# Ryan-Yanlong/DREAM-GNN

Hardware: AMD Instinct MI355X
Metric: GCMC+FGCN SpMM edges/sec and achieved HBM GB/s at 1/2/4/8 MI355X (higher is better)
Workload: dtype f32

## Files before the change

### dream_gnn_amd/csrc/dgmi_api.hip

```cpp
#include <hip/hip_runtime.h>
#include <limits.h>
#include <stdlib.h>
#include <string.h>

#include "dgmi.h"
#include "dgmi_bf16.h"
#include "dgmi_keep.h"
#include "dgmi_kernels.h"
#include "dgmi_tuning.h"

namespace {

inline hipStream_t as_stream(dgmi_stream_t s) { return static_cast<hipStream_t>(s); }

inline int from_hip(hipError_t e) { return e == hipSuccess ? DGMI_OK : DGMI_ERR_LAUNCH; }

long long env_ll(const char* name, long long dflt) {
  const char* e = getenv(name);
  return e != nullptr && e[0] != '\0' ? atoll(e) : dflt;
}

}

namespace dgmi {

Tuning& tuning() {
  static Tuning t = [] {
    Tuning v;
    v.sliced_rows = (int)env_ll("DGMI_SLICED_ROWS", 0);
    v.sliced_touch_lead = (int)env_ll("DGMI_SLICED_PF", -1);
    v.sliced_lpr = (int)env_ll("DGMI_SLICED_LPR", 0);
    v.sliced_no_off32 = getenv("DGMI_NO_OFF32") != nullptr ? 1 : 0;
    v.sliced_chunk_rows = env_ll("DGMI_SLICED_CHUNK_ROWS", 0);
    v.sliced_taper_rows = env_ll("DGMI_SLICED_TAPER_ROWS", 0);
    v.sliced_owned = (int)env_ll("DGMI_SLICED_OWNED", -1);
    v.sliced_owned_grid = (int)env_ll("DGMI_SLICED_OWNED_GRID", 0);
    v.sliced_owned_wgs = (int)env_ll("DGMI_SLICED_OWNED_WGS", 0);
    v.sliced_owned_rows = (int)env_ll("DGMI_SLICED_OWNED_ROWS", 0);
    v.sliced_owned_lds_rows = env_ll("DGMI_SLICED_OWNED_LDS_ROWS", 0);
    v.sliced_owned_lag = (int)env_ll("DGMI_SLICED_OWNED_LAG", -2);
    v.sliced_owned_spin_ticks = env_ll("DGMI_SLICED_OWNED_SPIN_TICKS", 0);
    v.select_window_min = env_ll("DGMI_SELECT_WINDOW_MIN", 0);
    v.select_narrow_window = env_ll("DGMI_SELECT_NARROW_WINDOW", 0) != 0 ? 1 : 0;
    v.sort_plain_tiles = env_ll("DGMI_SORT_PLAIN_TILES", 0) != 0 ? 1 : 0;
    v.knn_screen_first = env_ll("DGMI_KNN_SCREEN_V1", 0) != 0 ? 1 : 0;
    v.knn_pool_chunks = env_ll("DGMI_KNN_POOL_CHUNKS", 0);
    return v;
  }();
  return t;
}

}

extern "C" {

DGMI_API int dgmi_set_tuning(const char* name, int64_t value) {
  if (name == nullptr) return DGMI_ERR_INVALID_ARG;
  dgmi::Tuning& t = dgmi::tuning();
  if (strcmp(name, "sliced_rows") == 0) t.sliced_rows = (int)value;
  else if (strcmp(name, "sliced_touch_lead") == 0) t.sliced_touch_lead = (int)value;
  else if (strcmp(name, "sliced_lpr") == 0) t.sliced_lpr = (int)value;
  else if (strcmp(name, "sliced_no_off32") == 0) t.sliced_no_off32 = value != 0;
  else if (strcmp(name, "sliced_chunk_rows") == 0) t.sliced_chunk_rows = value;
  else if (strcmp(name, "sliced_taper_rows") == 0) t.sliced_taper_rows = value;
  else if (strcmp(name, "sliced_owned") == 0) t.sliced_owned = (int)value;
  else if (strcmp(name, "sliced_owned_grid") == 0) t.sliced_owned_grid = (int)value;
  else if (strcmp(name, "sliced_owned_wgs") == 0) t.sliced_owned_wgs = (int)value;
  else if (strcmp(name, "sliced_owned_rows") == 0) t.sliced_owned_rows = (int)value;
  else if (strcmp(name, "sliced_owned_lds_rows") == 0) t.sliced_owned_lds_rows = value;
  else if (strcmp(name, "sliced_owned_lag") == 0) t.sliced_owned_lag = (int)value;
  else if (strcmp(name, "sliced_owned_spin_ticks") == 0) t.sliced_owned_spin_ticks = value;
  else if (strcmp(name, "select_window_min") == 0) t.select_window_min = value;
  else if (strcmp(name, "select_narrow_window") == 0) t.select_narrow_window = value != 0;
  else if (strcmp(name, "sort_plain_tiles") == 0) t.sort_plain_tiles = value != 0;
  else if (strcmp(name, "knn_screen_first") == 0) t.knn_screen_first = value != 0;
  else if (strcmp(name, "knn_pool_chunks") == 0) t.knn_pool_chunks = value;
  else return DGMI_ERR_INVALID_ARG;
  return DGMI_OK;
}

DGMI_API int dgmi_abi_version(void) { return DGMI_ABI_VERSION; }

DGMI_API const char* dgmi_status_string(int status) {
  switch (status) {
    case DGMI_OK: return "ok";
    case DGMI_ERR_INVALID_ARG: return "invalid argument (null pointer, negative size or ld < F)";
    case DGMI_ERR_TOO_LARGE: return "size does not fit the int32 id space";
    case DGMI_ERR_WORKSPACE: return "workspace missing or too small";
    case DGMI_ERR_LAUNCH: return "HIP launch failed";
    case DGMI_ERR_NO_DEVICE: return "no gfx950 device visible";
    default: return "unknown dgmi status";
  }
}

DGMI_API int dgmi_device_ok(void) {
  int n = 0;
  if (hipGetDeviceCount(&n) != hipSuccess || n <= 0) return 0;
  int dev = 0;
  if (hipGetDevice(&dev) != hipSuccess) return 0;
  hipDeviceProp_t prop;
  if (hipGetDeviceProperties(&prop, dev) != hipSuccess) return 0;
  return strncmp(prop.gcnArchName, "gfx950", 6) == 0 ? 1 : 0;
}

DGMI_API int dgmi_csr_from_coo_i32(const int32_t* row, const int32_t* col, int64_t E, int64_t n_rows,
                          int64_t n_cols, int32_t* indptr, int32_t* indices, int32_t* eid, void* workspace,
                          size_t* workspace_bytes, dgmi_stream_t stream) {
  if (E < 0 || n_rows < 0 || workspace_bytes == nullptr) return DGMI_ERR_INVALID_ARG;
  if (E > INT32_MAX || n_rows >= INT32_MAX || n_cols >= INT32_MAX) return DGMI_ERR_TOO_LARGE;
  if (workspace != nullptr) {
    if (indptr == nullptr) return DGMI_ERR_INVALID_ARG;
    if (E > 0 && (row == nullptr || col == nullptr || indices == nullptr || eid == nullptr))
      return DGMI_ERR_INVALID_ARG;
  }
  size_t need = 0;
  hipError_t err = dgmi::csr_from_coo_i32(row, col, E, n_rows, n_cols, indptr, indices, eid, nullptr,
                                          &need, as_stream(stream));
  if (err != hipSuccess) return DGMI_ERR_LAUNCH;
  if (workspace == nullptr) {
    *workspace_bytes = need;
    return DGMI_OK;
  }
  if (*workspace_bytes < need) return DGMI_ERR_WORKSPACE;
  return from_hip(dgmi::csr_from_coo_i32(row, col, E, n_rows, n_cols, indptr, indices, eid, workspace,
                                         workspace_bytes, as_stream(stream)));
}

static bool epilogue_ok(int32_t act, const float* out_mask, int64_t ld_mask, int64_t F) {
  return (act == 0 || act == 1) && (out_mask == nullptr || ld_mask >= F);
}

static bool keep_args_ok(const int32_t* eid, const uint32_t* keep, int32_t n_keep) {
  if (n_keep < 0 || n_keep > dgmi::kMaxKeepSegs) return false;
  return n_keep == 0 || (eid != nullptr && keep != nullptr);
}

DGMI_API int dgmi_spmm_csr_f32(const int32_t* indptr, const int32_t* indices, const float* vals,
                      const int32_t* eid, const uint32_t* keep, int32_t n_keep,
                      const float* X, int64_t ldx, const float* src_scale,
                      const float* dst_scale, float* Y, int64_t ldy, int64_t n_dst,
                      int64_t n_src, int64_t F, int32_t act, float act_slope, const float* out_mask,
                      int64_t ld_mask, float out_mask_scale, dgmi_stream_t stream) {
  if (n_dst < 0 || n_src < 0 || F < 0 || !keep_args_ok(eid, keep, n_keep) || !epilogue_ok(act, out_mask, ld_mask, F))
    return DGMI_ERR_INVALID_ARG;
  if (n_dst >= INT32_MAX || n_src >= INT32_MAX || F > INT32_MAX) return DGMI_ERR_TOO_LARGE;
  if (n_dst == 0 || F == 0) return DGMI_OK;
  if (indptr == nullptr || Y == nullptr) return DGMI_ERR_INVALID_ARG;
  if (ldx < F || ldy < F) return DGMI_ERR_INVALID_ARG;
  if (X == nullptr && n_src > 0) return DGMI_ERR_INVALID_ARG;
  if (static_cast<const void*>(X) == static_cast<const void*>(Y)) return DGMI_ERR_INVALID_ARG;
  dgmi::SpmmArgs a{indptr, indices, vals, X, ldx, src_scale, dst_scale, Y, ldy, n_dst, n_src, F,
                   nullptr, 0, 0, nullptr, 0, eid, keep, n_keep, {act, act_slope, out_mask, ld_mask, out_mask_scale}};
  return from_hip(dgmi::spmm_csr_f32(a, as_stream(stream)));
}

DGMI_API int32_t dgmi_spmm_default_chunk(int64_t n_rows, int64_t nnz) {
  (void)n_rows;
  int64_t c = (nnz / 4096 + 63) / 64 * 64;
  if (c < 64) c = 64;
  if (c > 512) c = 512;
  return (int32_t)c;
}

static bool chunk_ok(int32_t chunk) { return chunk >= 16 && chunk <= 65536; }

DGMI_API size_t dgmi_spmm_plan_bytes(int64_t n_rows, int64_t nnz, int32_t chunk) {
  if (n_rows < 0 || nnz < 0 || !chunk_ok(chunk)) return 0;
  return dgmi::plan_bytes(n_rows, nnz, chunk);
}

DGMI_API size_t dgmi_spmm_partials_bytes(int64_t nnz, int32_t chunk, int64_t F) {
  if (nnz < 0 || F < 0 || !chunk_ok(chunk)) return 0;
  const size_t ldp = (size_t)((F + 3) / 4 * 4);
  const size_t b = (size_t)dgmi::plan_slots_cap(nnz, chunk) * ldp * sizeof(float);
  return b < 16 ? 16 : b;
}

DGMI_API int dgmi_spmm_plan_build(const int32_t* indptr, int64_t n_rows, int64_t nnz, int32_t chunk,
                                  void* plan, size_t plan_bytes, void* workspace,
                                  size_t* workspace_bytes, dgmi_stream_t stream) {
  if (n_rows < 0 || nnz < 0 || !chunk_ok(chunk) || workspace_bytes == nullptr)
    return DGMI_ERR_INVALID_ARG;
  if (n_rows >= INT32_MAX || nnz > INT32_MAX) return DGMI_ERR_TOO_LARGE;
  size_t need = 0;
  if (dgmi::spmm_plan_build(indptr, n_rows, nnz, chunk, nullptr, nullptr, &need, as_stream(stream)) !=
      hipSuccess)
    return DGMI_ERR_LAUNCH;
  if (workspace == nullptr) {
    *workspace_bytes = need;
    return DGMI_OK;
  }
  if (plan == nullptr || (indptr == nullptr && n_rows > 0)) return DGMI_ERR_INVALID_ARG;
  if (*workspace_bytes < need || plan_bytes < dgmi::plan_bytes(n_rows, nnz, chunk))
    return DGMI_ERR_WORKSPACE;
  return from_hip(dgmi::spmm_plan_build(indptr, n_rows, nnz, chunk, static_cast<int32_t*>(plan),
                                        workspace, workspace_bytes, as_stream(stream)));
}

DGMI_API int dgmi_spmm_csr_planned_f32(const int32_t* indptr, const int32_t* indices,
                                       const float* vals, const int32_t* eid, const uint32_t* keep,
                                       int32_t n_keep, const float* X, int64_t ldx,
                                       const float* src_scale, const float* dst_scale, float* Y,
                                       int64_t ldy, int64_t n_dst, int64_t n_src, int64_t F,
                                       int64_t nnz, int32_t chunk, const void* plan, void* partials,
                                       size_t partials_bytes, int32_t act, float act_slope,
                                       const float* out_mask, int64_t ld_mask, float out_mask_scale,
                                       dgmi_stream_t stream) {
  if (n_dst < 0 || n_src < 0 || F < 0 || nnz < 0 || !chunk_ok(chunk) || !keep_args_ok(eid, keep, n_keep) ||
      !epilogue_ok(act, out_mask, ld_mask, F))
    return DGMI_ERR_INVALID_ARG;
  if (n_dst >= INT32_MAX || n_src >= INT32_MAX || F > INT32_MAX || nnz > INT32_MAX)
    return DGMI_ERR_TOO_LARGE;
  if (n_dst == 0 || F == 0) return DGMI_OK;
  if (indptr == nullptr || Y == nullptr || plan == nullptr || partials == nullptr)
    return DGMI_ERR_INVALID_ARG;
  if (ldx < F || ldy < F) return DGMI_ERR_INVALID_ARG;
  if (X == nullptr && n_src > 0) return DGMI_ERR_INVALID_ARG;
  if (static_cast<const void*>(X) == static_cast<const void*>(Y)) return DGMI_ERR_INVALID_ARG;
  if (partials_bytes < dgmi_spmm_partials_bytes(nnz, chunk, F)) return DGMI_ERR_WORKSPACE;
  dgmi::SpmmArgs a{indptr, indices, vals, X, ldx, src_scale, dst_scale, Y, ldy, n_dst, n_src, F,
                   static_cast<const int32_t*>(plan), nnz, chunk, static_cast<float*>(partials),
                   (F + 3) / 4 * 4, eid, keep, n_keep, {act, act_slope, out_mask, ld_mask, out_mask_scale}};
// ... 336 lines not shown
```

### dream_gnn_amd/csrc/dgmi_owned.hip

```cpp
#include <hip/hip_runtime.h>
#include <stdint.h>

#include <map>
#include <mutex>
#include <utility>

#include "dgmi_owned_common.h"
#include "dgmi_sliced_common.h"

namespace dgmi {
namespace {

constexpr int kOwnedTouchChunk = 4;
constexpr int kOwnedTouchLead = 8;
constexpr int64_t kOwnedSpinTicks = 3000;
constexpr int64_t kOwnedMinRows = 32768;
constexpr int kOwnedLag = -1;

struct OwnedWork {
  int phase, task, slice, col_round;
  int64_t row0;
  int lds_row, rows;
};

__device__ __forceinline__ OwnedWork owned_decode(const OwnedPlan& pl, int64_t wg, int T, int k, int grp) {
  OwnedWork w;
  w.phase = k / T;
  w.task = k - w.phase * T;
  const OwnedPhase ph = owned_phase(pl, w.phase);
  w.slice = ph.slice;
  w.col_round = ph.col_round;
  const OwnedTask t = owned_task(pl, wg, ph.row_round, w.task, grp);
  w.row0 = t.row0;
  w.lds_row = t.lds_row;
  w.rows = t.rows;
  return w;
}

template <int LPR, int VALS, bool OFF32, int WAVES>
__global__ __launch_bounds__(kWave* WAVES, WAVES == kOwnedWaves ? 4 : 6) void spmm_owned_kernel(
    const int32_t* __restrict__ segptr, const int32_t* __restrict__ indices, const float* __restrict__ X, int64_t ldx,
    const float* __restrict__ dst_scale, float* __restrict__ Y, int64_t ldy, int64_t n_dst, int F, OwnedPlan pl,
    unsigned* __restrict__ arrive, int lag, int64_t spin_ticks, Epilogue ep) {
  constexpr bool MULT = VALS == 2;
  constexpr int kIdMask = MULT ? (int)kMultIdMask : 0x7fffffff;
  extern __shared__ float4 lds_rows[];
  const int lane = threadIdx.x & (kWave - 1);
  const int wave = threadIdx.x >> 6;
  const int grp = lane / LPR, glane = lane % LPR, gbase = grp * LPR;
  const int64_t wg = blockIdx.x;
  const int T = owned_wg_tasks(pl, wg);
  if (T == 0) return;
  int* done = reinterpret_cast<int*>(lds_rows + (size_t)pl.round_rows * LPR);
  int* phase_cnt = done + pl.tasks;
  int* counter = phase_cnt + pl.phases;
  int* open = counter + 1;
  for (int i = threadIdx.x; i < pl.tasks + pl.phases + 2; i += blockDim.x) done[i] = 0;
  __syncthreads();
  const int total = pl.phases * T;
  const int label = (int)(blockIdx.x & 7u);

  if (wave == WAVES - 1) {
    const unsigned n_label = (unsigned)((pl.active - label + 7) >> 3);
    const unsigned* my_arrive = arrive + (size_t)label * pl.phases;
    const int chunks_per_phase = (T + kOwnedTouchChunk - 1) / kOwnedTouchChunk, chunks = pl.phases * chunks_per_phase;
    const int last_gate = lag >= 0 ? pl.phases - 1 : 0;
    int keepalive = 0, touched = 0, opened = 0;
    bool waiting = false;
    uint64_t wait_start = 0;
    while (touched < chunks || opened < last_gate) {
      bool idle = true;
      const int next = __hip_atomic_load(counter, __ATOMIC_RELAXED, __HIP_MEMORY_SCOPE_WORKGROUP);
      if (touched < chunks) {
        const int P = touched / chunks_per_phase, t0 = (touched - P * chunks_per_phase) * kOwnedTouchChunk;
        if (P * T + t0 <= next + kOwnedTouchLead) {
          ++touched;
          idle = false;
          const OwnedPhase ph = owned_phase(pl, P);
          const int64_t in_round = owned_round_rows(pl, wg, ph.row_round);
          const int64_t lds_first = (int64_t)t0 * pl.G * pl.R;
          int64_t lds_last = lds_first + (int64_t)kOwnedTouchChunk * pl.G * pl.R;
          if (lds_last > in_round) lds_last = in_round;
          if (lds_first < lds_last) {
            const int32_t* sp_s = segptr + (int64_t)ph.slice * n_dst;
            const int64_t r_first = owned_task(pl, wg, ph.row_round, t0, 0).row0, r_last = r_first + (lds_last - lds_first);
            const int64_t rp = lane == 0 ? r_first : (lane == 1 ? r_last : r_first + (int64_t)(lane - 1) * 32);
            int v = 0;
            if (rp <= r_last) v = sp_s[rp];
            keepalive ^= v;
            const int e0 = __builtin_amdgcn_readlane(v, 0), e1 = __builtin_amdgcn_readlane(v, 1);
            for (int64_t p = (int64_t)e0 + (int64_t)lane * 32; p < e1; p += (int64_t)kWave * 32) keepalive ^= indices[p];
            asm volatile("" ::"v"(keepalive));
          }
        }
      }
      if (opened < last_gate) {
        const int P = opened + 1, need = P - 1 - lag;
        bool ok = need < 0 || __hip_atomic_load(&my_arrive[need], __ATOMIC_RELAXED, __HIP_MEMORY_SCOPE_AGENT) >= n_label;
        if (!ok && next >= P * T) {
          const uint64_t now = __builtin_amdgcn_s_memrealtime();
          if (!waiting) {
            waiting = true;
            wait_start = now;
          } else if (now - wait_start >= (uint64_t)spin_ticks) {
            ok = true;
          }
        }
        if (ok) {
          opened = P;
          waiting = false;
          idle = false;
          __hip_atomic_store(open, P, __ATOMIC_RELAXED, __HIP_MEMORY_SCOPE_WORKGROUP);
        }
      }
      if (idle) __builtin_amdgcn_s_sleep(2);
    }
    return;
  }

  auto grab = [&]() {
    int k = 0;
    if (lane == 0) k = __hip_atomic_fetch_add(counter, 1, __ATOMIC_RELAXED, __HIP_MEMORY_SCOPE_WORKGROUP);
    return __builtin_amdgcn_readfirstlane(k);
  };
  auto boundaries = [&](int k) {
    if (k >= total) return 0;
    const OwnedWork w = owned_decode(pl, wg, T, k, grp);
    if (w.rows == 0) return 0;
    return segptr[(int64_t)w.slice * n_dst + w.row0 + (glane < w.rows ? glane : w.rows)];
  };
  auto first_ids = [&](int my_b, int rows, int batch) {
    const int e_begin = __shfl(my_b, gbase, kWave), e_end = __shfl(my_b, gbase + rows, kWave);
    if (rows == 0 || e_begin >= e_end) return 0;
    return indices[e_begin + owned_window_id_edge(batch, glane, e_end - e_begin)];
  };
  static_assert(kOwnedWindowFirstBatches == 2, "nxt_idx and nxt_idx1");

  const uint32_t row_bytes = (uint32_t)ldx * 4u;
  int k = grab();
  int my_b = boundaries(k);
  int nxt_idx = k < total ? first_ids(my_b, owned_decode(pl, wg, T, k, grp).rows, 0) : 0;
  int nxt_idx1 = k < total ? first_ids(my_b, owned_decode(pl, wg, T, k, grp).rows, 1) : 0;
  while (k < total) {
    const OwnedWork w = owned_decode(pl, wg, T, k, grp);
    const int k_next = grab();
    const int next_b = boundaries(k_next);
    if (lag >= 0)
      while (__hip_atomic_load(open, __ATOMIC_RELAXED, __HIP_MEMORY_SCOPE_WORKGROUP) < w.phase) __builtin_amdgcn_s_sleep(1);
    while (__hip_atomic_load(&done[w.task], __ATOMIC_ACQUIRE, __HIP_MEMORY_SCOPE_WORKGROUP) < w.phase) __builtin_amdgcn_s_sleep(1);

    const int nr = w.rows;
    int col = (w.col_round * LPR + glane) * 4;
    const bool col_ok = col < F;
    if (!col_ok) col = 0;
    const float* Xc = X + col;
    const uint32_t col_bytes = (uint32_t)col * 4u;
    float4* slot = lds_rows + (size_t)w.lds_row * LPR + glane;
    auto commit = [&](int r, const float4& acc) {
      if (w.slice == 0) {
        slot[r * LPR] = acc;
        return;
      }
      float4 t = slot[r * LPR];
      t.x += acc.x;
      t.y += acc.y;
      t.z += acc.z;
      t.w += acc.w;
      slot[r * LPR] = t;
    };
    auto write_rows = [&]() {
      if (w.slice != kOwnedSlices - 1 || !col_ok) return;
      for (int r = 0; r < nr; ++r) {
        float4 t = slot[r * LPR];
        const int64_t row = w.row0 + r;
        if (dst_scale != nullptr) {
          const float d = dst_scale[row];
          t.x *= d;
          t.y *= d;
          t.z *= d;
          t.w *= d;
        }
        *reinterpret_cast<float4*>(Y + row * ldy + col) = epilogue4(ep, t, row, col);
      }
    };

    if (nr > 0) {
      const int e_begin = __shfl(my_b, gbase, kWave);
      const int e_end = __shfl(my_b, gbase + nr, kWave);
      int r = 0;
      int row_end = __shfl(my_b, gbase + 1, kWave);
      float4 acc = make_float4(0.f, 0.f, 0.f, 0.f);
      if (e_begin < e_end) {
        constexpr int W = kOwnedWindow;
        static_assert(W <= 8 && kMultShift == 28 && LPR % W == 0, "at most eight 4-bit multiplicity fields, shifted down from bit 28");
        const int L = e_end - e_begin;
        float4 v[W];
        int idx[W];
        uint32_t mults = 0, mults_in = 0;
        auto read_ids = [&](int batch_idx) {
#pragma unroll
          for (int u = 0; u < W; ++u) {
            int id = __shfl(batch_idx, gbase + u, kWave);
            if (MULT) {
              mults_in = (mults_in >> 4) | ((uint32_t)id & ((uint32_t)kMultMax << kMultShift));
              id &= kIdMask;
            }
            idx[u] = id;
          }
          if (MULT) asm volatile("" : "+v"(mults_in));
        };
        auto add = [&](int u) {
          if (MULT) {
            const float m = (float)(((mults >> (32 - 4 * W)) & (uint32_t)kMultMax) + 1u);
            mults >>= 4;
            acc.x = fmaf(m, v[u].x, acc.x);
            acc.y = fmaf(m, v[u].y, acc.y);
            acc.z = fmaf(m, v[u].z, acc.z);
            acc.w = fmaf(m, v[u].w, acc.w);
          } else {
            acc.x += v[u].x;
            acc.y += v[u].y;
            acc.z += v[u].z;
            acc.w += v[u].w;
          }
        };
        auto rows_before = [&](int p) {
          while (p >= row_end) {
            commit(r, acc);
            acc = make_float4(0.f, 0.f, 0.f, 0.f);
            ++r;
            row_end = __shfl(my_b, gbase + r + 1, kWave);
          }
        };
        read_ids(nxt_idx);
        int ids = nxt_idx1;
#pragma unroll
        for (int u = 0; u < W; ++u) v[u] = ld_row<OFF32>(X, Xc, idx[u], ldx, row_bytes, col_bytes);
        mults = mults_in;
        __builtin_amdgcn_sched_barrier(0);
        int p0 = e_begin;
        for (int g = 0; p0 + W < e_end; ++g, p0 += W) {
          read_ids(ids);
          ids = indices[e_begin + owned_window_id_edge(owned_window_request_batch(g), glane, L)];
          __builtin_amdgcn_sched_barrier(0);
#pragma unroll
          for (int u = 0; u < W; ++u) {
            rows_before(p0 + u);
            add(u);
            v[u] = ld_row<OFF32>(X, Xc, idx[u], ldx, row_bytes, col_bytes);
            __builtin_amdgcn_sched_barrier(0);
          }
          mults = mults_in;
        }
#pragma unroll
        for (int u = 0; u < W; ++u) {
          if (p0 + u < e_end) {
            rows_before(p0 + u);
            add(u);
          }
        }
      }
      for (; r < nr; ++r) {
        commit(r, acc);
        acc = make_float4(0.f, 0.f, 0.f, 0.f);
      }
      write_rows();
    }
    nxt_idx = k_next < total ? first_ids(next_b, owned_decode(pl, wg, T, k_next, grp).rows, 0) : 0;
    nxt_idx1 = k_next < total ? first_ids(next_b, owned_decode(pl, wg, T, k_next, grp).rows, 1) : 0;
    __builtin_amdgcn_wave_barrier();
    if (lane == 0) {
      __hip_atomic_store(&done[w.task], w.phase + 1, __ATOMIC_RELEASE, __HIP_MEMORY_SCOPE_WORKGROUP);
      if (lag >= 0) {
        const int finished = __hip_atomic_fetch_add(&phase_cnt[w.phase], 1, __ATOMIC_RELAXED, __HIP_MEMORY_SCOPE_WORKGROUP);
        if (finished == T - 1)
          __hip_atomic_fetch_add(&arrive[(size_t)label * pl.phases + w.phase], 1u, __ATOMIC_RELAXED, __HIP_MEMORY_SCOPE_AGENT);
      }
    }
    k = k_next;
    my_b = next_b;
  }
}

int device_cus() {
  static const int cus = [] {
    int dev = 0, n = 0;
    if (hipGetDevice(&dev) != hipSuccess || hipDeviceGetAttribute(&n, hipDeviceAttributeMultiprocessorCount, dev) != hipSuccess)
      return 0;
    return n;
  }();
  return cus;
}

int owned_class_form(const OwnedPlan& pl, bool id_mult, int64_t table_bytes) {
  const auto mib = [&](int64_t lo, int64_t hi) { return table_bytes >= (lo << 20) && table_bytes <= (hi << 20); };
  if (pl.col_rounds == 1 && pl.row_rounds == 2 && !id_mult && mib(16, 32)) return 1;
  if (pl.col_rounds == 2 && pl.row_rounds == 1 && id_mult && mib(48, 64)) return 1;
  if (pl.col_rounds == 1 && pl.row_rounds == 1 && id_mult && mib(16, 32)) return 1;
  return 0;
}

bool owned_coresident(const void* kern, int threads, size_t lds, int wgs) {
  static std::mutex mu;
  static std::map<std::pair<const void*, size_t>, int> known;
  std::lock_guard<std::mutex> lock(mu);
  auto it = known.find({kern, lds});
  if (it == known.end()) {
    int n = 0;
    if (hipOccupancyMaxActiveBlocksPerMultiprocessor(&n, kern, threads, lds) != hipSuccess) {
      (void)hipGetLastError();
      n = 0;
    }
    it = known.emplace(std::make_pair(kern, lds), n).first;
  }
  return it->second >= wgs;
}

template <int LPR, int WAVES>
hipError_t launch_owned(const SlicedArgs& a, const OwnedPlan& pl, int64_t grid, bool off32, int lag, int64_t spin_ticks,
                        hipStream_t s, bool* resident) {
  constexpr int kWgsPerCu = WAVES == kOwnedWaves ? 1 : 2;
  unsigned* arrive = reinterpret_cast<unsigned*>(a.planes);
  *resident = true;
#define DGMI_OWNED(V, O)                                                                                                  \
  do {                                                                                                                    \
    if constexpr (kWgsPerCu > 1 && LPR == 8 && V == 2) {                                                                  \
      *resident = false;                                                                                                  \
      return hipSuccess;                                                                                                  \
    } else {                                                                                                              \
    auto kern = spmm_owned_kernel<LPR, V, O, WAVES>;                                                                      \
    static const hipError_t attr = hipFuncSetAttribute(reinterpret_cast<const void*>(kern),                               \
                                                       hipFuncAttributeMaxDynamicSharedMemorySize, (160 << 10) / kWgsPerCu); \
    if (attr != hipSuccess) return attr;                                                                                  \
    if (kWgsPerCu > 1 && !owned_coresident(reinterpret_cast<const void*>(kern), kWave * WAVES, pl.lds_bytes, kWgsPerCu)) { \
      *resident = false;                                                                                                  \
      return hipSuccess;                                                                                                  \
    }                                                                                                                     \
    if (lag >= 0) {                                                            \
      const hipError_t err = hipMemsetAsync(arrive, 0, sizeof(unsigned) * 8 * (size_t)pl.phases, s);                      \
      if (err != hipSuccess) return err;                                                                                  \
    }                                                                                                                     \
    hipLaunchKernelGGL(kern, dim3((unsigned)grid), dim3(kWave* WAVES), pl.lds_bytes, s, a.segptr, a.indices,              \
                       static_cast<const float*>(a.X), a.ldx, a.dst_scale, a.Y, a.ldy, a.n_dst, (int)a.F, pl, arrive, lag, \
                       spin_ticks, a.ep);                                                                                 \
    }                                                                                                                     \
  } while (0)
  if (a.id_mult) {
    if (off32) DGMI_OWNED(2, true); else DGMI_OWNED(2, false);
  } else {
    if (off32) DGMI_OWNED(0, true); else DGMI_OWNED(0, false);
  }
#undef DGMI_OWNED
  return hipGetLastError();
}

}

hipError_t spmm_owned_try(const SlicedArgs& a, hipStream_t s, bool* taken) {
  *taken = false;
  const Tuning& tune = tuning();
  if (tune.sliced_owned == 0) return hipSuccess;
  if (a.x_bytes != 4 || a.vals != nullptr || a.src_scale != nullptr || a.n_keep != 0 || a.n_slices != kOwnedSlices ||
      tune.sliced_chunk_rows > 0 || a.chunk_rows < a.n_dst || a.n_dst == 0 || a.F == 0)
    return hipSuccess;
  const int64_t grid = tune.sliced_owned_grid > 0 ? tune.sliced_owned_grid : device_cus();
  if (grid < 1) return hipSuccess;
  const int lpr = sliced_lpr(a.F, a.n_src, a.n_slices, a.n_dst, a.full_width, a.n_keep, a.x_bytes, tune.sliced_lpr);
  const OwnedPlan pl = owned_plan(a.n_dst, a.F, lpr, grid, tune.sliced_owned_rows, tune.sliced_owned_lds_rows);
  if (!pl.ok || pl.lds_bytes > (size_t)(160 << 10)) return hipSuccess;
  const auto arrive_fits = [&](const OwnedPlan& p) {
    return sizeof(unsigned) * 8 * (size_t)p.phases <= sizeof(float) * (size_t)a.n_slices * (size_t)a.n_dst * (size_t)a.ldp;
  };
  if (!arrive_fits(pl)) return hipSuccess;
  const int rule = a.n_dst < kOwnedMinRows ? 0 : owned_class_form(pl, a.id_mult, a.n_src * a.ldx * (int64_t)sizeof(float));
  if (tune.sliced_owned != 1 && rule == 0) return hipSuccess;
  const int form = tune.sliced_owned_wgs == 1 || tune.sliced_owned_wgs == 2 ? tune.sliced_owned_wgs : (rule == 2 ? 2 : 1);
  const bool off32 = !tune.sliced_no_off32 && (a.n_src * a.ldx + a.F) * 4 < ((int64_t)1 << 32);
  const int64_t spin = tune.sliced_owned_spin_ticks > 0 ? tune.sliced_owned_spin_ticks : kOwnedSpinTicks;
  const int lag = tune.sliced_owned_lag >= -1 ? tune.sliced_owned_lag : kOwnedLag;
  *taken = true;
  bool resident = true;
  if (form == 2) {
    const int64_t grid2 = tune.sliced_owned_grid > 0 ? grid : 2 * grid;
    const OwnedPlan pl2 = owned_plan(a.n_dst, a.F, lpr, grid2, tune.sliced_owned_rows, tune.sliced_owned_lds_rows, 2);
    if (pl2.ok && pl2.lds_bytes <= (size_t)(80 << 10) && arrive_fits(pl2)) {
      hipError_t err;
      switch (lpr) {
        case 8: err = launch_owned<8, kOwnedPairWaves>(a, pl2, grid2, off32, lag, spin, s, &resident); break;
        case 16: err = launch_owned<16, kOwnedPairWaves>(a, pl2, grid2, off32, lag, spin, s, &resident); break;
        case 32: err = launch_owned<32, kOwnedPairWaves>(a, pl2, grid2, off32, lag, spin, s, &resident); break;
        default: err = launch_owned<64, kOwnedPairWaves>(a, pl2, grid2, off32, lag, spin, s, &resident); break;
      }
      if (err != hipSuccess || resident) return err;
    }
  }
  switch (lpr) {
    case 8: return launch_owned<8, kOwnedWaves>(a, pl, grid, off32, lag, spin, s, &resident);
    case 16: return launch_owned<16, kOwnedWaves>(a, pl, grid, off32, lag, spin, s, &resident);
    case 32: return launch_owned<32, kOwnedWaves>(a, pl, grid, off32, lag, spin, s, &resident);
    default: return launch_owned<64, kOwnedWaves>(a, pl, grid, off32, lag, spin, s, &resident);
  }
}

}
```

### dream_gnn_amd/csrc/dgmi_owned_common.h

```cpp
#pragma once
#include <hip/hip_runtime.h>
#include <stddef.h>
#include <stdint.h>

namespace dgmi {

constexpr int kOwnedSlices = 8;
constexpr int kOwnedWaves = 16;
constexpr int kOwnedWorkers = kOwnedWaves - 1;
constexpr int kOwnedPairWaves = 12;
constexpr int64_t kOwnedLdsRowBytes = 144 << 10;
constexpr int kOwnedMaxPhases = 128;
constexpr int kOwnedPhaseTasks = 24;
constexpr int kOwnedMaxRows = 8;

struct OwnedPlan {
  bool ok;
  int lpr, G, R;
  int col_rounds, row_rounds, phases;
  int64_t wg_rows;
  int64_t active;
  int round_rows;
  int tasks;
  int64_t n_dst;
  size_t lds_bytes;
};

struct OwnedPhase {
  int col_round, row_round, slice;
};

struct OwnedTask {
  int64_t row0;
  int lds_row;
  int rows;
};

__host__ __device__ constexpr int owned_form_waves(int wgs_per_cu) { return wgs_per_cu == 2 ? kOwnedPairWaves : kOwnedWaves; }

__host__ __device__ inline OwnedPlan owned_plan(int64_t n_dst, int64_t F, int lpr, int64_t grid, int R_req, int64_t lds_rows_cap,
                                                int wgs_per_cu = 1) {
  OwnedPlan p{};
  p.ok = false;
  p.n_dst = n_dst;
  if (n_dst < 1 || F < 1 || grid < 1 || (wgs_per_cu != 1 && wgs_per_cu != 2) || (lpr != 8 && lpr != 16 && lpr != 32 && lpr != 64)) return p;
  p.lpr = lpr;
  p.G = 64 / lpr;
  p.col_rounds = (int)((F + 4 * lpr - 1) / (4 * lpr));
  p.wg_rows = (n_dst + grid - 1) / grid;
  p.active = (n_dst + p.wg_rows - 1) / p.wg_rows;
  int64_t fit = kOwnedLdsRowBytes / wgs_per_cu / (16 * lpr);
  if (lds_rows_cap > 0 && lds_rows_cap < fit) fit = lds_rows_cap;
  const int64_t rounds = (p.wg_rows + fit - 1) / fit;
  if (rounds * p.col_rounds * kOwnedSlices > kOwnedMaxPhases) return p;
  p.row_rounds = (int)rounds;
  p.round_rows = (int)((p.wg_rows + rounds - 1) / rounds);
  p.phases = p.col_rounds * p.row_rounds * kOwnedSlices;
  int R = R_req;
  if (R <= 0) {
    const int phase_tasks = (kOwnedPhaseTasks * (owned_form_waves(wgs_per_cu) - 1) + kOwnedWorkers / 2) / kOwnedWorkers;
    R = (p.round_rows + phase_tasks * p.G / 2) / (phase_tasks * p.G);
    if (R > kOwnedMaxRows) R = kOwnedMaxRows;
  }
  if (R > lpr - 1) R = lpr - 1;
  if (R < 1) R = 1;
  p.R = R;
  p.tasks = (p.round_rows + p.G * R - 1) / (p.G * R);
  p.lds_bytes = (size_t)p.round_rows * 16 * lpr + sizeof(int) * ((size_t)p.tasks + p.phases + 2);
  p.ok = true;
  return p;
}

__host__ __device__ inline int64_t owned_wg_rows(const OwnedPlan& p, int64_t wg) {
  const int64_t left = p.n_dst - wg * p.wg_rows;
  return left < 0 ? 0 : (left < p.wg_rows ? left : p.wg_rows);
}

__host__ __device__ inline int64_t owned_round_rows(const OwnedPlan& p, int64_t wg, int row_round) {
  const int64_t left = owned_wg_rows(p, wg) - (int64_t)row_round * p.round_rows;
  return left < 0 ? 0 : (left < p.round_rows ? left : p.round_rows);
}

__host__ __device__ inline int owned_wg_tasks(const OwnedPlan& p, int64_t wg) {
  int64_t rows = owned_wg_rows(p, wg);
  if (rows > p.round_rows) rows = p.round_rows;
  return (int)((rows + p.G * p.R - 1) / (p.G * p.R));
}

__host__ __device__ inline OwnedPhase owned_phase(const OwnedPlan& p, int phase) {
  const int cq = phase / kOwnedSlices;
  return OwnedPhase{cq / p.row_rounds, cq % p.row_rounds, phase % kOwnedSlices};
}

__host__ __device__ inline OwnedTask owned_task(const OwnedPlan& p, int64_t wg, int row_round, int task, int group) {
  const int64_t lds_row = ((int64_t)task * p.G + group) * p.R;
  int64_t rows = owned_round_rows(p, wg, row_round) - lds_row;
  rows = rows < 0 ? 0 : (rows < p.R ? rows : p.R);
  return OwnedTask{wg * p.wg_rows + (int64_t)row_round * p.round_rows + lds_row, (int)lds_row, (int)rows};
}

constexpr int kOwnedWindow = 4;
constexpr int kOwnedWindowFirstBatches = 2;

__host__ __device__ constexpr int owned_window_groups(int L) { return (L + kOwnedWindow - 1) / kOwnedWindow; }

__host__ __device__ constexpr int owned_window_issue_batch(int g) { return g + 1; }
__host__ __device__ constexpr int owned_window_request_batch(int g) { return g + kOwnedWindowFirstBatches; }

__host__ __device__ constexpr int owned_window_id_edge(int batch, int lane, int L) {
  return batch * kOwnedWindow + lane % kOwnedWindow < L ? batch * kOwnedWindow + lane % kOwnedWindow : L - 1;
}

}
```

### dream_gnn_amd/csrc/dgmi_tuning.h

```cpp
#pragma once
#include <stdint.h>

namespace dgmi {

struct Tuning {
  int sliced_rows = 0;
  int sliced_touch_lead = -1;
  int sliced_lpr = 0;
  int sliced_no_off32 = 0;
  int64_t sliced_chunk_rows = 0;
  int64_t sliced_taper_rows = 0;
  int sliced_owned = -1;
  int sliced_owned_grid = 0;
  int sliced_owned_wgs = 0;
  int sliced_owned_rows = 0;
  int64_t sliced_owned_lds_rows = 0;
  int sliced_owned_lag = -2;
  int64_t sliced_owned_spin_ticks = 0;
  int64_t select_window_min = 0;
  int select_narrow_window = 0;
  int sort_plain_tiles = 0;
  int knn_screen_first = 0;
  int64_t knn_pool_chunks = 0;
};

Tuning& tuning();

}
```

Measured before the change: 36.35 billion.

## Carry next task's first gather window across tasks in owned SpMM kernel

In the owned SpMM kernel with multiplicity ids, each worker wave now decodes the next task early and issues the first window of X row loads for it during the tail of the current task. This hides the gather latency at task boundaries. The dst_scale values are also prefetched through shuffles instead of being loaded per row. Separately, a larger per-phase task target is selected for certain table-size and plan classes, and an optional env knob caps the number of worker waves. The change adds register pressure and more complex control flow, and it only applies to the single-WG-per-CU multiplicity path.

```diff
diff --git a/dream_gnn_amd/csrc/dgmi_api.hip b/dream_gnn_amd/csrc/dgmi_api.hip
--- a/dream_gnn_amd/csrc/dgmi_api.hip
+++ b/dream_gnn_amd/csrc/dgmi_api.hip
@@ -38,6 +38,7 @@
     v.sliced_owned_wgs = (int)env_ll("DGMI_SLICED_OWNED_WGS", 0);
     v.sliced_owned_rows = (int)env_ll("DGMI_SLICED_OWNED_ROWS", 0);
     v.sliced_owned_lds_rows = env_ll("DGMI_SLICED_OWNED_LDS_ROWS", 0);
+    v.sliced_owned_workers = (int)env_ll("DGMI_SLICED_OWNED_WORKERS", 0);
     v.sliced_owned_lag = (int)env_ll("DGMI_SLICED_OWNED_LAG", -2);
     v.sliced_owned_spin_ticks = env_ll("DGMI_SLICED_OWNED_SPIN_TICKS", 0);
     v.select_window_min = env_ll("DGMI_SELECT_WINDOW_MIN", 0);
@@ -68,6 +69,7 @@
   else if (strcmp(name, "sliced_owned_wgs") == 0) t.sliced_owned_wgs = (int)value;
   else if (strcmp(name, "sliced_owned_rows") == 0) t.sliced_owned_rows = (int)value;
   else if (strcmp(name, "sliced_owned_lds_rows") == 0) t.sliced_owned_lds_rows = value;
+  else if (strcmp(name, "sliced_owned_workers") == 0) t.sliced_owned_workers = (int)value;
   else if (strcmp(name, "sliced_owned_lag") == 0) t.sliced_owned_lag = (int)value;
   else if (strcmp(name, "sliced_owned_spin_ticks") == 0) t.sliced_owned_spin_ticks = value;
   else if (strcmp(name, "select_window_min") == 0) t.select_window_min = value;
diff --git a/dream_gnn_amd/csrc/dgmi_owned.hip b/dream_gnn_amd/csrc/dgmi_owned.hip
--- a/dream_gnn_amd/csrc/dgmi_owned.hip
+++ b/dream_gnn_amd/csrc/dgmi_owned.hip
@@ -19,19 +19,25 @@
 
 struct OwnedWork {
   int phase, task, slice, col_round;
-  int64_t row0;
+  int64_t row_base;
   int lds_row, rows;
 };
 
 __device__ __forceinline__ OwnedWork owned_decode(const OwnedPlan& pl, int64_t wg, int T, int k, int grp) {
   OwnedWork w;
+  if (k >= pl.phases * T) {
+    w.phase = pl.phases;
+    w.task = w.slice = w.col_round = w.lds_row = w.rows = 0;
+    w.row_base = 0;
+    return w;
+  }
   w.phase = k / T;
   w.task = k - w.phase * T;
   const OwnedPhase ph = owned_phase(pl, w.phase);
   w.slice = ph.slice;
   w.col_round = ph.col_round;
   const OwnedTask t = owned_task(pl, wg, ph.row_round, w.task, grp);
-  w.row0 = t.row0;
+  w.row_base = t.row0 - t.lds_row;
   w.lds_row = t.lds_row;
   w.rows = t.rows;
   return w;
@@ -41,9 +47,10 @@
 __global__ __launch_bounds__(kWave* WAVES, WAVES == kOwnedWaves ? 4 : 6) void spmm_owned_kernel(
     const int32_t* __restrict__ segptr, const int32_t* __restrict__ indices, const float* __restrict__ X, int64_t ldx,
     const float* __restrict__ dst_scale, float* __restrict__ Y, int64_t ldy, int64_t n_dst, int F, OwnedPlan pl,
-    unsigned* __restrict__ arrive, int lag, int64_t spin_ticks, Epilogue ep) {
+    unsigned* __restrict__ arrive, int lag, int64_t spin_ticks, int workers, Epilogue ep) {
   constexpr bool MULT = VALS == 2;
   constexpr int kIdMask = MULT ? (int)kMultIdMask : 0x7fffffff;
+  constexpr bool CARRY = WAVES == kOwnedWaves && MULT;
   extern __shared__ float4 lds_rows[];
   const int lane = threadIdx.x & (kWave - 1);
   const int wave = threadIdx.x >> 6;
@@ -118,43 +125,86 @@
     return;
   }
 
+  if (workers > 0 && wave >= workers) return;
   auto grab = [&]() {
     int k = 0;
     if (lane == 0) k = __hip_atomic_fetch_add(counter, 1, __ATOMIC_RELAXED, __HIP_MEMORY_SCOPE_WORKGROUP);
     return __builtin_amdgcn_readfirstlane(k);
   };
-  auto boundaries = [&](int k) {
-    if (k >= total) return 0;
-    const OwnedWork w = owned_decode(pl, wg, T, k, grp);
-    if (w.rows == 0) return 0;
-    return segptr[(int64_t)w.slice * n_dst + w.row0 + (glane < w.rows ? glane : w.rows)];
-  };
-  auto first_ids = [&](int my_b, int rows, int batch) {
-    const int e_begin = __shfl(my_b, gbase, kWave), e_end = __shfl(my_b, gbase + rows, kWave);
-    if (rows == 0 || e_begin >= e_end) return 0;
-    return indices[e_begin + owned_window_id_edge(batch, glane, e_end - e_begin)];
-  };
+  auto boundaries = [&](const OwnedWork& t) {
+    return segptr[t.rows == 0 ? 0 : (int64_t)t.slice * n_dst + t.row_base + (t.lds_row + (glane < t.rows ? glane : t.rows))];
+  };
+  auto scales = [&](const OwnedWork& t) {
+    if (!CARRY || dst_scale == nullptr || t.slice != kOwnedSlices - 1 || t.rows == 0) return 0.f;
+    return dst_scale[t.row_base + (t.lds_row + (glane < t.rows ? glane : t.rows - 1))];
+  };
+  int nxt_idx = 0, nxt_idx1 = 0, rel_b = 0;
+  float my_ds = 0.f, nxt_ds = 0.f;
   static_assert(kOwnedWindowFirstBatches == 2, "nxt_idx and nxt_idx1");
+  auto hand_over = [&](int b, const OwnedWork& nxt, int& beg, int& end) {
+    beg = __shfl(b, gbase, kWave);
+    rel_b = b - beg;
+    end = beg + __shfl(rel_b, gbase + nxt.rows, kWave);
+    if (beg < end) {
+      nxt_idx = indices[beg + owned_carry_slot_edge(glane % kOwnedWindow, end - beg)];
+      nxt_idx1 = indices[beg + owned_window_id_edge(owned_carry_start_batch(), glane, end - beg)];
+    }
+    my_ds = nxt_ds;
+    nxt_ds = scales(nxt);
+  };
+
+  constexpr int W = kOwnedWindow;
+  static_assert(W <= 8 && kMultShift == 28 && LPR % W == 0, "at most eight 4-bit multiplicity fields, shifted down from bit 28");
+  float4 v[W];
+  int idx[W];
+  int nidx[W];
+  uint32_t mults = 0, mults_in = 0, nmults = 0;
+  bool carried = false;
+  auto read_batch = [&](int batch_idx, int (&out)[W], uint32_t& fields) {
+#pragma unroll
+    for (int u = 0; u < W; ++u) {
+      int id = __shfl(batch_idx, gbase + u, kWave);
+      if (MULT) {
+        fields = (fields >> 4) | ((uint32_t)id & ((uint32_t)kMultMax << kMultShift));
+        id &= kIdMask;
+      }
+      out[u] = id;
+    }
+    if (MULT) asm volatile("" : "+v"(fields));
+  };
+  auto read_ids = [&](int batch_idx) { read_batch(batch_idx, idx, mults_in); };
 
   const uint32_t row_bytes = (uint32_t)ldx * 4u;
   int k = grab();
-  int my_b = boundaries(k);
-  int nxt_idx = k < total ? first_ids(my_b, owned_decode(pl, wg, T, k, grp).rows, 0) : 0;
-  int nxt_idx1 = k < total ? first_ids(my_b, owned_decode(pl, wg, T, k, grp).rows, 1) : 0;
+  OwnedWork w = owned_decode(pl, wg, T, k, grp);
+  int e_begin = 0, e_end = 0;
+  hand_over(boundaries(w), w, e_begin, e_end);
+  int my_rel = rel_b;
   while (k < total) {
-    const OwnedWork w = owned_decode(pl, wg, T, k, grp);
-    const int k_next = grab();
-    const int next_b = boundaries(k_next);
-    if (lag >= 0)
-      while (__hip_atomic_load(open, __ATOMIC_RELAXED, __HIP_MEMORY_SCOPE_WORKGROUP) < w.phase) __builtin_amdgcn_s_sleep(1);
-    while (__hip_atomic_load(&done[w.task], __ATOMIC_ACQUIRE, __HIP_MEMORY_SCOPE_WORKGROUP) < w.phase) __builtin_amdgcn_s_sleep(1);
-
-    const int nr = w.rows;
+    const int L = e_end - e_begin;
     int col = (w.col_round * LPR + glane) * 4;
     const bool col_ok = col < F;
     if (!col_ok) col = 0;
     const float* Xc = X + col;
     const uint32_t col_bytes = (uint32_t)col * 4u;
+    if (L > 0 && !carried) {
+      read_ids(nxt_idx);
+#pragma unroll
+      for (int u = 0; u < W; ++u) v[u] = ld_row<OFF32>(X, Xc, idx[u], ldx, row_bytes, col_bytes);
+      mults = mults_in;
+    }
+    const int k_next = grab();
+    const OwnedWork w_next = owned_decode(pl, wg, T, k_next, grp);
+    const int next_b = boundaries(w_next);
+    int n_begin = 0, n_end = 0;
+    if (lag >= 0)
+      while (__hip_atomic_load(open, __ATOMIC_RELAXED, __HIP_MEMORY_SCOPE_WORKGROUP) < w.phase) __builtin_amdgcn_s_sleep(1);
+    while (__hip_atomic_load(&done[w.task], __ATOMIC_ACQUIRE, __HIP_MEMORY_SCOPE_WORKGROUP) < w.phase) __builtin_amdgcn_s_sleep(1);
+    const int first_ids = nxt_idx1;
+    static_assert(owned_carry_start_batch() == 1, "nxt_idx1");
+    if (CARRY) hand_over(next_b, w_next, n_begin, n_end);
+
+    const int nr = w.rows;
     float4* slot = lds_rows + (size_t)w.lds_row * LPR + glane;
     auto commit = [&](int r, const float4& acc) {
       if (w.slice == 0) {
@@ -169,12 +219,15 @@
       slot[r * LPR] = t;
     };
     auto write_rows = [&]() {
-      if (w.slice != kOwnedSlices - 1 || !col_ok) return;
+      if (w.slice != kOwnedSlices - 1) return;
       for (int r = 0; r < nr; ++r) {
+        float d = 0.f;
+        if (CARRY) d = __shfl(my_ds, gbase + r, kWave);
+        if (!col_ok) continue;
         float4 t = slot[r * LPR];
-        const int64_t row = w.row0 + r;
+        const int64_t row = w.row_base + (w.lds_row + r);
         if (dst_scale != nullptr) {
-          const float d = dst_scale[row];
+          if (!CARRY) d = dst_scale[row];
           t.x *= d;
           t.y *= d;
           t.z *= d;
@@ -184,90 +237,108 @@
       }
     };
 
-    if (nr > 0) {
-      const int e_begin = __shfl(my_b, gbase, kWave);
-      const int e_end = __shfl(my_b, gbase + nr, kWave);
-      int r = 0;
-      int row_end = __shfl(my_b, gbase + 1, kWave);
-      float4 acc = make_float4(0.f, 0.f, 0.f, 0.f);
-      if (e_begin < e_end) {
-        constexpr int W = kOwnedWindow;
-        static_assert(W <= 8 && kMultShift == 28 && LPR % W == 0, "at most eight 4-bit multiplicity fields, shifted down from bit 28");
-        const int L = e_end - e_begin;
-        float4 v[W];
-        int idx[W];
-        uint32_t mults = 0, mults_in = 0;
-        auto read_ids = [&](int batch_idx) {
+    bool carry = false;
+    int r = 0;
+    float4 acc = make_float4(0.f, 0.f, 0.f, 0.f);
+    if (L > 0) {
+      int row_end = e_begin + __shfl(my_rel, gbase + 1, kWave);
+      auto add = [&](int u) {
+        if (MULT) {
+          const float m = (float)(((mults >> (32 - 4 * W)) & (uint32_t)kMultMax) + 1u);
+          mults >>= 4;
+          acc.x = fmaf(m, v[u].x, acc.x);
+          acc.y = fmaf(m, v[u].y, acc.y);
+          acc.z = fmaf(m, v[u].z, acc.z);
+          acc.w = fmaf(m, v[u].w, acc.w);
+        } else {
+          acc.x += v[u].x;
+          acc.y += v[u].y;
+          acc.z += v[u].z;
+          acc.w += v[u].w;
+        }
+      };
+      auto rows_before = [&](int p) {
+        while (p >= row_end) {
+          commit(r, acc);
+          acc = make_float4(0.f, 0.f, 0.f, 0.f);
+          ++r;
+          row_end = e_begin + __shfl(my_rel, gbase + r + 1, kWave);
+        }
+      };
+      int ids = first_ids;
+      __builtin_amdgcn_sched_barrier(0);
+      int p0 = e_begin;
+      carry = CARRY && owned_carry(L, n_end - n_begin);
+      auto group = [&](int g) {
+        read_ids(ids);
+        ids = indices[e_begin + owned_window_id_edge(owned_window_request_batch(g), glane, L)];
+        __builtin_amdgcn_sched_barrier(0);
 #pragma unroll
-          for (int u = 0; u < W; ++u) {
-            int id = __shfl(batch_idx, gbase + u, kWave);
-            if (MULT) {
-              mults_in = (mults_in >> 4) | ((uint32_t)id & ((uint32_t)kMultMax << kMultShift));
-              id &= kIdMask;
-            }
-            idx[u] = id;
-          }
-          if (MULT) asm volatile("" : "+v"(mults_in));
-        };
-        auto add = [&](int u) {
-          if (MULT) {
-            const float m = (float)(((mults >> (32 - 4 * W)) & (uint32_t)kMultMax) + 1u);
-            mults >>= 4;
-            acc.x = fmaf(m, v[u].x, acc.x);
-            acc.y = fmaf(m, v[u].y, acc.y);
-            acc.z = fmaf(m, v[u].z, acc.z);
-            acc.w = fmaf(m, v[u].w, acc.w);
-          } else {
-            acc.x += v[u].x;
-            acc.y += v[u].y;
-            acc.z += v[u].z;
-            acc.w += v[u].w;
-          }
-        };
-        auto rows_before = [&](int p) {
-          while (p >= row_end) {
-            commit(r, acc);
-            acc = make_float4(0.f, 0.f, 0.f, 0.f);
-            ++r;
-            row_end = __shfl(my_b, gbase + r + 1, kWave);
-          }
-        };
-        read_ids(nxt_idx);
-        int ids = nxt_idx1;
-#pragma unroll
-        for (int u = 0; u < W; ++u) v[u] = ld_row<OFF32>(X, Xc, idx[u], ldx, row_bytes, col_bytes);
+        for (int u = 0; u < W; ++u) {
+          rows_before(p0 + u);
+          add(u);
+          v[u] = ld_row<OFF32>(X, Xc, idx[u], ldx, row_bytes, col_bytes);
+          __builtin_amdgcn_sched_barrier(0);
+        }
         mults = mults_in;
-        __builtin_amdgcn_sched_barrier(0);
-        int p0 = e_begin;
-        for (int g = 0; p0 + W < e_end; ++g, p0 += W) {
-          read_ids(ids);
-          ids = indices[e_begin + owned_window_id_edge(owned_window_request_batch(g), glane, L)];
-          __builtin_amdgcn_sched_barrier(0);
-#pragma unroll
-          for (int u = 0; u < W; ++u) {
-            rows_before(p0 + u);
-            add(u);
-            v[u] = ld_row<OFF32>(X, Xc, idx[u], ldx, row_bytes, col_bytes);
-            __builtin_amdgcn_sched_barrier(0);
-          }
-          mults = mults_in;
-        }
+      };
+      static_assert(owned_carry_read_group(2 * W + 1) == 0 && owned_carry_read_group(2 * W) == -1, "behind group 0 of three or more");
+      int g = 0;
+      if (owned_carry_read_group(L) == 0) {
+        group(0);
+        p0 += W;
+        if (carry) read_batch(nxt_idx, nidx, nmults);
+        group(1);
+        p0 += W;
+        g = 2;
+      } else {
+        if (p0 + W < e_end) {
+          group(0);
+          p0 += W;
+          g = 1;
+        }
+        if (carry) read_batch(nxt_idx, nidx, nmults);
+      }
+      for (; p0 + W < e_end; ++g, p0 += W) group(g);
+      const float* Xn = X;
+      uint32_t ncol_bytes = 0;
+      if (carry) {
+        int ncol = (w_next.col_round * LPR + glane) * 4;
+        if (ncol >= F) ncol = 0;
+        Xn = X + ncol;
+        ncol_bytes = (uint32_t)ncol * 4u;
+      }
+      __builtin_amdgcn_sched_barrier(0);
+      if (carry) {
 #pragma unroll
         for (int u = 0; u < W; ++u) {
           if (p0 + u < e_end) {
             rows_before(p0 + u);
             add(u);
           }
-        }
-      }
+          v[u] = ld_row<OFF32>(X, Xn, nidx[u], ldx, row_bytes, ncol_bytes);
+          __builtin_amdgcn_sched_barrier(0);
+        }
+        mults = nmults;
+      } else {
+#pragma unroll
+        for (int u = 0; u < W; ++u) {
+          if (p0 + u < e_end) {
+            rows_before(p0 + u);
+            add(u);
+          }
+        }
+      }
+    }
+    if (nr > 0) {
       for (; r < nr; ++r) {
         commit(r, acc);
         acc = make_float4(0.f, 0.f, 0.f, 0.f);
       }
       write_rows();
     }
-    nxt_idx = k_next < total ? first_ids(next_b, owned_decode(pl, wg, T, k_next, grp).rows, 0) : 0;
-    nxt_idx1 = k_next < total ? first_ids(next_b, owned_decode(pl, wg, T, k_next, grp).rows, 1) : 0;
+    const OwnedWork w_then = CARRY ? w_next : owned_decode(pl, wg, T, k_next, grp);
+    if (!CARRY) hand_over(next_b, w_then, n_begin, n_end);
     __builtin_amdgcn_wave_barrier();
     if (lane == 0) {
       __hip_atomic_store(&done[w.task], w.phase + 1, __ATOMIC_RELEASE, __HIP_MEMORY_SCOPE_WORKGROUP);
@@ -278,7 +349,11 @@
       }
     }
     k = k_next;
-    my_b = next_b;
+    w = w_then;
+    my_rel = rel_b;
+    e_begin = n_begin;
+    e_end = n_end;
+    carried = carry;
   }
 }
 
@@ -298,6 +373,13 @@
   if (pl.col_rounds == 2 && pl.row_rounds == 1 && id_mult && mib(48, 64)) return 1;
   if (pl.col_rounds == 1 && pl.row_rounds == 1 && id_mult && mib(16, 32)) return 1;
   return 0;
+}
+
+int owned_class_phase_tasks(const OwnedPlan& pl, bool id_mult, int64_t table_bytes) {
+  const auto mib = [&](int64_t lo, int64_t hi) { return table_bytes >= (lo << 20) && table_bytes <= (hi << 20); };
+  if (pl.col_rounds == 2 && pl.row_rounds == 1 && id_mult && mib(48, 64)) return kOwnedPhaseTasksMult;
+  if (pl.col_rounds == 1 && pl.row_rounds == 1 && id_mult && mib(16, 32)) return kOwnedPhaseTasksMult;
+  return kOwnedPhaseTasks;
 }
 
 bool owned_coresident(const void* kern, int threads, size_t lds, int wgs) {
@@ -321,6 +403,7 @@
                         hipStream_t s, bool* resident) {
   constexpr int kWgsPerCu = WAVES == kOwnedWaves ? 1 : 2;
   unsigned* arrive = reinterpret_cast<unsigned*>(a.planes);
+  const int workers = tuning().sliced_owned_workers > 0 && tuning().sliced_owned_workers < WAVES - 1 ? tuning().sliced_owned_workers : 0;
   *resident = true;
 #define DGMI_OWNED(V, O)                                                                                                  \
   do {                                                                                                                    \
@@ -342,7 +425,7 @@
     }                                                                                                                     \
     hipLaunchKernelGGL(kern, dim3((unsigned)grid), dim3(kWave* WAVES), pl.lds_bytes, s, a.segptr, a.indices,              \
                        static_cast<const float*>(a.X), a.ldx, a.dst_scale, a.Y, a.ldy, a.n_dst, (int)a.F, pl, arrive, lag, \
-                       spin_ticks, a.ep);                                                                                 \
+                       spin_ticks, workers, a.ep);                                                                               \
     }                                                                                                                     \
   } while (0)
   if (a.id_mult) {
@@ -366,7 +449,11 @@
   const int64_t grid = tune.sliced_owned_grid > 0 ? tune.sliced_owned_grid : device_cus();
   if (grid < 1) return hipSuccess;
   const int lpr = sliced_lpr(a.F, a.n_src, a.n_slices, a.n_dst, a.full_width, a.n_keep, a.x_bytes, tune.sliced_lpr);
-  const OwnedPlan pl = owned_plan(a.n_dst, a.F, lpr, grid, tune.sliced_owned_rows, tune.sliced_owned_lds_rows);
+  OwnedPlan pl = owned_plan(a.n_dst, a.F, lpr, grid, tune.sliced_owned_rows, tune.sliced_owned_lds_rows);
+  const int phase_tasks = a.n_dst < kOwnedMinRows ? kOwnedPhaseTasks
+                                                   : owned_class_phase_tasks(pl, a.id_mult, a.n_src * a.ldx * (int64_t)sizeof(float));
+  if (pl.ok && phase_tasks != kOwnedPhaseTasks)
+    pl = owned_plan(a.n_dst, a.F, lpr, grid, tune.sliced_owned_rows, tune.sliced_owned_lds_rows, 1, phase_tasks);
   if (!pl.ok || pl.lds_bytes > (size_t)(160 << 10)) return hipSuccess;
   const auto arrive_fits = [&](const OwnedPlan& p) {
     return sizeof(unsigned) * 8 * (size_t)p.phases <= sizeof(float) * (size_t)a.n_slices * (size_t)a.n_dst * (size_t)a.ldp;
diff --git a/dream_gnn_amd/csrc/dgmi_owned_common.h b/dream_gnn_amd/csrc/dgmi_owned_common.h
--- a/dream_gnn_amd/csrc/dgmi_owned_common.h
+++ b/dream_gnn_amd/csrc/dgmi_owned_common.h
@@ -12,6 +12,7 @@
 constexpr int64_t kOwnedLdsRowBytes = 144 << 10;
 constexpr int kOwnedMaxPhases = 128;
 constexpr int kOwnedPhaseTasks = 24;
+constexpr int kOwnedPhaseTasksMult = 32;
 constexpr int kOwnedMaxRows = 8;
 
 struct OwnedPlan {
@@ -39,7 +40,7 @@
 __host__ __device__ constexpr int owned_form_waves(int wgs_per_cu) { return wgs_per_cu == 2 ? kOwnedPairWaves : kOwnedWaves; }
 
 __host__ __device__ inline OwnedPlan owned_plan(int64_t n_dst, int64_t F, int lpr, int64_t grid, int R_req, int64_t lds_rows_cap,
-                                                int wgs_per_cu = 1) {
+                                                int wgs_per_cu = 1, int phase_tasks_target = kOwnedPhaseTasks) {
   OwnedPlan p{};
   p.ok = false;
   p.n_dst = n_dst;
@@ -58,7 +59,7 @@
   p.phases = p.col_rounds * p.row_rounds * kOwnedSlices;
   int R = R_req;
   if (R <= 0) {
-    const int phase_tasks = (kOwnedPhaseTasks * (owned_form_waves(wgs_per_cu) - 1) + kOwnedWorkers / 2) / kOwnedWorkers;
+    const int phase_tasks = (phase_tasks_target * (owned_form_waves(wgs_per_cu) - 1) + kOwnedWorkers / 2) / kOwnedWorkers;
     R = (p.round_rows + phase_tasks * p.G / 2) / (phase_tasks * p.G);
     if (R > kOwnedMaxRows) R = kOwnedMaxRows;
   }
@@ -111,4 +112,12 @@
   return batch * kOwnedWindow + lane % kOwnedWindow < L ? batch * kOwnedWindow + lane % kOwnedWindow : L - 1;
 }
 
+__host__ __device__ constexpr bool owned_carry(int L_a, int L_b) { return L_a > 0 && L_b > 0; }
+
+__host__ __device__ constexpr int owned_carry_slot_edge(int u, int L_b) { return owned_window_id_edge(0, u, L_b); }
+
+__host__ __device__ constexpr int owned_carry_read_group(int L_a) { return owned_window_groups(L_a) >= 3 ? 0 : -1; }
+
+__host__ __device__ constexpr int owned_carry_start_batch() { return owned_window_issue_batch(0); }
+
 }
diff --git a/dream_gnn_amd/csrc/dgmi_tuning.h b/dream_gnn_amd/csrc/dgmi_tuning.h
--- a/dream_gnn_amd/csrc/dgmi_tuning.h
+++ b/dream_gnn_amd/csrc/dgmi_tuning.h
@@ -15,6 +15,7 @@
   int sliced_owned_wgs = 0;
   int sliced_owned_rows = 0;
   int64_t sliced_owned_lds_rows = 0;
+  int sliced_owned_workers = 0;
   int sliced_owned_lag = -2;
   int64_t sliced_owned_spin_ticks = 0;
   int64_t select_window_min = 0;
```

Result: faster. 36.76 billion, median of 6 (+1.1%).
